# DCASE-REPO/DESED_task

Measured on AMD Instinct MI355X. Metric: 10s-clips/sec CRNN mean-teacher train @batch48, higher is better.
Workload: dtype f32 (fp32 storage and accumulation; the dense contractions of the wide layers run as split-bf16 MFMA, 3 bf16 products per fp32 product, fp32-level accuracy; everything else exact f32)

## Files before the change

### desed_task_amd/_lib.py

```python
import ctypes
import os
import re

_HERE = os.path.dirname(os.path.abspath(__file__))
_HEADER = os.path.join(os.path.dirname(_HERE), "include", "sed_hip.h")
LIB_PATH = os.path.join(_HERE, "libsed_hip.so")

_CTYPES = {"int": ctypes.c_int, "float": ctypes.c_float, "double": ctypes.c_double, "long long": ctypes.c_longlong,
           "unsigned": ctypes.c_uint, "unsigned int": ctypes.c_uint}

ERRORS = {-1: "bad argument", -2: "kernel launch failed", -3: "unsupported configuration"}


def parse_header(path=_HEADER):
    text = open(path).read()
    text = re.sub(r"/\*.*?\*/", "", text, flags=re.S)
    protos = {}
    for m in re.finditer(r"\b(?:int|long long)\s+(sed_\w+)\s*\(([^)]*)\)\s*;", text):
        args = []
        for a in m.group(2).split(","):
            a = a.strip()
            if "*" in a:
                args.append(ctypes.c_void_p)
            else:
                ty = re.sub(r"\bconst\b", "", a).strip()
                ty = ty.rsplit(None, 1)[0].strip()
                args.append(_CTYPES[ty])
        protos[m.group(1)] = args
    return protos


def header_constants(path=_HEADER):
    return {m.group(1): int(m.group(2)) for m in re.finditer(r"^#define\s+(SED_\w+)\s+(\d+)\b", open(path).read(), re.M)}


class _Lib:
    def __init__(self, path, is_emulator=False):
        self.path = path
        self.is_emulator = is_emulator
        import torch
        self._dll = ctypes.CDLL(path)
        self.protos = parse_header()
        for name, argtypes in self.protos.items():
            fn = getattr(self._dll, name)
            fn.argtypes = argtypes
            fn.restype = ctypes.c_longlong if name.endswith("_floats") else ctypes.c_int

    def value(self, name, *args):
        return getattr(self._dll, name)(*args)

    def call(self, name, *args):
        rc = getattr(self._dll, name)(*args)
        if rc != 0:
            raise RuntimeError("%s failed: %s (rc=%d)" % (name, ERRORS.get(rc, "?"), rc))


_lib = None


def get():
    global _lib
    if _lib is None:
        if not os.path.exists(LIB_PATH):
            raise RuntimeError(
                "desed_task_amd: %s is missing -- build it with `python -m desed_task_amd.build` "
                "(hipcc --offload-arch=gfx950).  There is no CPU fallback." % LIB_PATH)
        _lib = _Lib(LIB_PATH)
    return _lib


def use_library(path, is_emulator=True):
    global _lib
    _lib = _Lib(path, is_emulator=is_emulator) if path is not None else None
    return _lib


TUNING_KEYS = {"glu_grid_cap": 0, "glu_bwd128_split": 1, "convb_ck": 2, "convb_mp": 3, "block0_nocenter": 4, "glu_fwd128": 5, "wgrad_narrow": 6, "wgrad_cap": 7, "attn_valu": 8, "wgrad_wide": 9, "gru_lds_kb": 10, "mel_taps_mem": 11, "convb_tpw": 12, "mel_wave": 13, "gemm_ntn": 14, "linear_tiles": 15}


_tuning = {}


def set_tuning(key, value):
    get().call("sed_set_tuning", TUNING_KEYS[key], int(value))
    _tuning[key] = int(value)


def get_tuning(key):
    return _tuning.get(key, 0)


def check_tensor(t, name="tensor"):
    lib = get()
    if lib.is_emulator:
        if t.is_cuda:
            raise RuntimeError("%s: emulator build bound but tensor is on the GPU" % name)
    elif not t.is_cuda:
        raise RuntimeError("%s must live on the MI355X (cuda) device: there is no CPU path" % name)
    if not t.is_contiguous():
        raise RuntimeError("%s must be contiguous" % name)


def stream_ptr(t):
    if t.is_cuda:
        import torch
        return torch.cuda.current_stream(t.device).cuda_stream
    return 0
```

### desed_task_amd/csrc/sed_common.h

```cpp
#pragma once

#ifdef SED_EMU
#include "hip_emu.h"
#else
#include <hip/hip_runtime.h>
#define SED_DYN_SMEM(name) extern __shared__ __attribute__((aligned(16))) char name[]
#define SED_LAUNCH(kern, grid, block, smem, stream, ...) \
    hipLaunchKernelGGL(kern, grid, block, smem, stream, __VA_ARGS__)
typedef float f32x16 __attribute__((ext_vector_type(16)));
typedef float f32x4 __attribute__((ext_vector_type(4)));
typedef short s16x8 __attribute__((ext_vector_type(8)));
#endif

#include <stdint.h>

#define SED_API extern "C" __attribute__((visibility("default")))

#define SED_MAX_SMEM(kern, bytes) \
    (void)hipFuncSetAttribute((const void*)(kern), hipFuncAttributeMaxDynamicSharedMemorySize, (int)(bytes))

__global__ __launch_bounds__(256) static void sed_zero4_kernel(float* p0, int n0, float* p1, int n1, float* p2, int n2, float* p3, int n3) {
    const int i = blockIdx.x * 256 + threadIdx.x;
    if (i < n0) p0[i] = 0.f;
    if (i < n1) p1[i] = 0.f;
    if (i < n2) p2[i] = 0.f;
    if (i < n3) p3[i] = 0.f;
}
static inline void sed_zero4(hipStream_t s, float* p0, int n0, float* p1, int n1, float* p2, int n2, float* p3, int n3) {
    int n = n0 > n1 ? n0 : n1;
    n = n > n2 ? n : n2;
    n = n > n3 ? n : n3;
    if (n <= 0) return;
    SED_LAUNCH(sed_zero4_kernel, dim3((n + 255) / 256), dim3(256), 0, s, p0, n0, p1, n1, p2, n2, p3, n3);
}

#define SED_OK 0
#define SED_ERR_ARG (-1)
#define SED_ERR_LAUNCH (-2)
#define SED_ERR_UNSUPPORTED (-3)

enum { SED_TUNE_GLU_GRID_CAP = 0, SED_TUNE_GLU_BWD128_SPLIT = 1, SED_TUNE_CONVB_CK = 2, SED_TUNE_CONVB_MP = 3, SED_TUNE_B0_NOCENTER = 4, SED_TUNE_GLU_FWD128 = 5, SED_TUNE_WGRAD_NARROW = 6, SED_TUNE_WGRAD_CAP = 7,
       SED_TUNE_ATTN_VALU = 8, SED_TUNE_WGRAD_WIDE = 9, SED_TUNE_GRU_LDS_KB = 10, SED_TUNE_MEL_TAPS_MEM = 11, SED_TUNE_CONVB_TPW = 12, SED_TUNE_MEL_WAVE = 13, SED_TUNE_GEMM_NTN = 14, SED_TUNE_LINEAR_TILES = 15, SED_TUNE_COUNT = 16 };
extern int sed_tuning[SED_TUNE_COUNT];

static inline int sed_check_launch() {
    hipError_t e = hipGetLastError();
    return e == hipSuccess ? SED_OK : SED_ERR_LAUNCH;
}

__device__ __forceinline__ f32x16 mfma32(float a, float b, f32x16 c) {
#ifdef SED_EMU
    return emu_mfma_32x32x2(a, b, c);
#else
    return __builtin_amdgcn_mfma_f32_32x32x2f32(a, b, c, 0, 0, 0);
#endif
}
__device__ __forceinline__ int mfma32_row(int r, int lane) { return (r & 3) + 8 * (r >> 2) + 4 * (lane >> 5); }

__device__ __forceinline__ f32x4 mfma16(float a, float b, f32x4 c) {
#ifdef SED_EMU
    return emu_mfma_16x16x4(a, b, c);
#else
    return __builtin_amdgcn_mfma_f32_16x16x4f32(a, b, c, 0, 0, 0);
#endif
}

__device__ __forceinline__ f32x16 mfma32_bf16(s16x8 a, s16x8 b, f32x16 c) {
#ifdef SED_EMU
    return emu_mfma_32x32x16_bf16(a, b, c);
#else
    typedef __bf16 bf16x8_t __attribute__((ext_vector_type(8)));
    return __builtin_amdgcn_mfma_f32_32x32x16_bf16(__builtin_bit_cast(bf16x8_t, a), __builtin_bit_cast(bf16x8_t, b), c, 0, 0, 0);
#endif
}
__device__ __forceinline__ f32x4 mfma16_bf16(s16x8 a, s16x8 b, f32x4 c) {
#ifdef SED_EMU
    return emu_mfma_16x16x32_bf16(a, b, c);
#else
    typedef __bf16 bf16x8_t __attribute__((ext_vector_type(8)));
    return __builtin_amdgcn_mfma_f32_16x16x32_bf16(__builtin_bit_cast(bf16x8_t, a), __builtin_bit_cast(bf16x8_t, b), c, 0, 0, 0);
#endif
}
__device__ __forceinline__ unsigned short f32_to_bf16(float x) {
    unsigned u = __float_as_uint(x);
    u += 0x7FFFu + ((u >> 16) & 1u);
    return (unsigned short)(u >> 16);
}
__device__ __forceinline__ float bf16_to_f32(unsigned short h) { return __uint_as_float(((unsigned)h) << 16); }
__device__ __forceinline__ void bf16_split(float x, unsigned short& hi, unsigned short& lo) {
    hi = f32_to_bf16(x);
    lo = f32_to_bf16(x - bf16_to_f32(hi));
}

__device__ __forceinline__ float sed_sadd(float a, float b) {
#ifdef SED_EMU
    return a + b;
// ... 308 lines not shown
```

### desed_task_amd/csrc/sed_conv.hip

```cpp
#include "sed_common.h"

__global__ __launch_bounds__(256) void pack_weights_kernel(const float* __restrict__ W, float* __restrict__ Wf,
                                                           float* __restrict__ Wd, int COUT, int CIN) {
    const int i = blockIdx.x * 256 + threadIdx.x;
    if (i >= COUT * CIN * 9) return;
    const int b = i % 3, a = (i / 3) % 3, ci = (i / 9) % CIN, co = i / (9 * CIN);
    const float w = W[i];
    Wf[((a * 3 + b) * CIN + ci) * COUT + co] = w;
    if (Wd) Wd[(((2 - a) * 3 + (2 - b)) * COUT + co) * CIN + ci] = w;
}
SED_API int sed_conv_pack_weights(const float* W, float* Wf, float* Wd, int COUT, int CIN, void* stream) {
    const int n = COUT * CIN * 9;
    SED_LAUNCH(pack_weights_kernel, dim3((n + 255) / 256), dim3(256), 0, (hipStream_t)stream, W, Wf, Wd, COUT, CIN);
    return sed_check_launch();
}
struct PackJobs {
    const float* W[8];
    float* Wf[8];
    float* Wd[8];
    int cout[8], cin[8], start[9];
    int n;
};
__global__ __launch_bounds__(256) void pack_weights_multi_kernel(PackJobs jobs) {
    const int i = blockIdx.x * 256 + threadIdx.x;
// ... 983 lines not shown
            for (int idx = tid; idx < ntp * CIN * COUT; idx += 256) part[(size_t)g0 * CIN * COUT + idx] = red[idx];
        }
        return;
    }
#pragma unroll
    for (int g0 = 0; g0 < 9; g0 += TG) {
        for (int round = 0; round < WK; ++round) {
            __syncthreads();
            if (wk == round) {
#pragma unroll
                for (int tp = g0; tp < g0 + TG && tp < 9; ++tp)
#pragma unroll
                    for (int n = 0; n < NTW; ++n) {
                        const int co = (wn * NTW + n) * 32 + lo;
#pragma unroll
                        for (int r = 0; r < 16; ++r) {
                            const int ci = mfma32_row(r, lane);
                            if (ci < CIN) {
                                float* d = red + ((tp - g0) * CIN + ci) * COUT + co;
                                *d = (round == 0) ? acc[tp][n][r] : *d + acc[tp][n][r];
                            }
                        }
                    }
            }
        }
        __syncthreads();
        const int ntp = (9 - g0) < TG ? (9 - g0) : TG;
        for (int idx = tid; idx < ntp * CIN * COUT; idx += 256) part[(size_t)g0 * CIN * COUT + idx] = red[idx];
    }
}
template <int CIN, int COUT, int TF>
static int launch_wgrad_alltaps(const float* x, const float* dy, float* dWp, int B, int T, int F, hipStream_t s) {
    using Cfg = WgaCfg<CIN, COUT, TF>;
    const int grid = wgrad_parts(CIN, COUT, B, T, F);
    SED_MAX_SMEM((conv_wgrad_alltaps_kernel<CIN, COUT, TF>), Cfg::SMEM);
    SED_LAUNCH((conv_wgrad_alltaps_kernel<CIN, COUT, TF>), dim3(grid), dim3(256), Cfg::SMEM, s, x, dy, dWp, B, T, F);
    return sed_check_launch();
}

#ifndef WGN_ABL
#define WGN_ABL 0
#endif
template <int CIN, int COUT>
struct WgnCfg {
    static constexpr int TF = 32, TR = 4, PH = TR + 2;
    static constexpr bool M16 = CIN == 16;
    static constexpr int XS = PH * TF + (M16 ? 16 : 8), DS = TR * TF + (M16 ? 16 : 8);
    static constexpr int XPLANE = CIN * XS, DPLANE = COUT * DS;
    static constexpr int SMEM_OPS = (6 * XPLANE + 2 * DPLANE) * 2, SMEM_RED = 9 * CIN * COUT * 4;
    static constexpr int SMEM = SMEM_OPS > SMEM_RED ? SMEM_OPS : SMEM_RED;
};
template <int CIN, int COUT>
__global__ __launch_bounds__(256) void conv_wgrad_alltaps_bf16_kernel(const float* __restrict__ x, const float* __restrict__ dy,
                                                                      float* __restrict__ dWp, int B, int T, int F) {
    using Cfg = WgnCfg<CIN, COUT>;
    constexpr int TF = Cfg::TF, TR = Cfg::TR, PH = Cfg::PH, XS = Cfg::XS, DS = Cfg::DS, XPLANE = Cfg::XPLANE, DPLANE = Cfg::DPLANE;
    constexpr bool M16 = Cfg::M16;
    static_assert((CIN == 16 && COUT == 32) || (CIN == 32 && COUT == 64), "the two narrow layers of the recipe");
    SED_DYN_SMEM(smem);
    unsigned short* xp = (unsigned short*)smem;
    unsigned short* dp = xp + 6 * XPLANE;
    const int lane = threadIdx.x & 63, w = threadIdx.x >> 6;
    int tid = threadIdx.x, lo = lane & 31, hi = lane >> 5, i16 = lane & 15, g = lane >> 4;
    const int ftiles = F / TF, ttiles = (T + TR - 1) / TR, ntiles = B * ttiles * ftiles;

    f32x16 acc[M16 ? 1 : 9];
    f32x4 acc16[M16 ? 9 : 1][2];
#pragma unroll
    for (int tp = 0; tp < (M16 ? 1 : 9); ++tp) acc[tp] = f32x16_zero();
#pragma unroll
    for (int tp = 0; tp < (M16 ? 9 : 1); ++tp) { acc16[tp][0] = f32x4{0.f, 0.f, 0.f, 0.f}; acc16[tp][1] = f32x4{0.f, 0.f, 0.f, 0.f}; }

    constexpr int VX = CIN / 4, VD = COUT / 4, NXI = PH * 8 * VX, NDI = TR * 8 * VD;
    constexpr int NXU = (NXI + 255) / 256, NDU = NDI / 256;
    float4 lx[NXU][6], ld[NDU][4];
    unsigned long long okx = 0;
    unsigned okd = 0;
    static_assert(NXU * 6 <= 64 && NDU <= 32, "validity masks");
    auto load_tile = [&](int tile_) {
        const int ft = tile_ % ftiles, tt = (tile_ / ftiles) % ttiles, b = tile_ / (ftiles * ttiles);
        const int t0 = tt * TR, f0 = ft * TF;
        okx = 0; okd = 0;
#pragma unroll
        for (int u = 0; u < NXU; ++u) {
            const int it = tid + 256 * u, cq = it % 8, v = (it / 8) % VX, i = it / (8 * VX);
            const int t = t0 - 1 + i;
            const bool rowok = it < NXI && t >= 0 && t < T && !(WGN_ABL & 8);
            const float* src = x + (((size_t)b * T + (t < 0 ? 0 : (t >= T ? T - 1 : t))) * F) * CIN + 4 * v;
#pragma unroll
            for (int k = 0; k < 6; ++k) {
                const int f = f0 - 1 + 4 * cq + k;
                okx |= (unsigned long long)((rowok && f >= 0 && f < F) ? 1 : 0) << (6 * u + k);
                lx[u][k] = *(const float4*)(src + (size_t)(f < 0 ? 0 : (f >= F ? F - 1 : f)) * CIN);
            }
        }
#pragma unroll
        for (int u = 0; u < NDU; ++u) {
            const int it = tid + 256 * u, cq = it % 8, v = (it / 8) % VD, r = it / (8 * VD);
            const int t = t0 + r;
            okd |= ((t < T && !(WGN_ABL & 8)) ? 1u : 0u) << u;
            const float* src = dy + (((size_t)b * T + (t < T ? t : T - 1)) * F + f0 + 4 * cq) * COUT + 4 * v;
#pragma unroll
            for (int k = 0; k < 4; ++k) ld[u][k] = *(const float4*)(src + (size_t)k * COUT);
        }
    };
    auto comp = [](const float4& q, int c) { return c == 0 ? q.x : c == 1 ? q.y : c == 2 ? q.z : q.w; };
    auto store_tile = [&]() {
#pragma unroll
        for (int u = 0; u < NXU; ++u)
#pragma unroll
            for (int k = 0; k < 6; ++k) if (!((okx >> (6 * u + k)) & 1ull)) lx[u][k] = make_float4(0.f, 0.f, 0.f, 0.f);
#pragma unroll
        for (int u = 0; u < NDU; ++u)
            if (!((okd >> u) & 1u)) {
#pragma unroll
                for (int k = 0; k < 4; ++k) ld[u][k] = make_float4(0.f, 0.f, 0.f, 0.f);
            }
#pragma unroll
        for (int u = 0; u < NXU; ++u) {
            const int it = tid + 256 * u, cq = it % 8, v = (it / 8) % VX, i = it / (8 * VX);
            if (it < NXI) {
#pragma unroll
                for (int c = 0; c < 4; ++c) {
                    unsigned ph[5], pl[5];
#pragma unroll
                    for (int k = 0; k < 5; ++k) bf16_split2(comp(lx[u][k], c), comp(lx[u][k + 1], c), ph[k], pl[k]);
                    unsigned short* dst = xp + (4 * v + c) * XS + i * TF + 4 * cq;
#pragma unroll
                    for (int sft = 0; sft < 3; ++sft) {
                        uint2 hv, lv;
                        hv.x = ph[sft]; hv.y = ph[sft + 2];
                        lv.x = pl[sft]; lv.y = pl[sft + 2];
                        *(uint2*)(dst + (2 * sft) * XPLANE) = hv;
                        *(uint2*)(dst + (2 * sft + 1) * XPLANE) = lv;
                    }
                }
            }
        }
#pragma unroll
        for (int u = 0; u < NDU; ++u) {
            const int it = tid + 256 * u, cq = it % 8, v = (it / 8) % VD, r = it / (8 * VD);
#pragma unroll
            for (int c = 0; c < 4; ++c) {
                uint2 hv, lv;
                bf16_split2(comp(ld[u][0], c), comp(ld[u][1], c), hv.x, lv.x);
                bf16_split2(comp(ld[u][2], c), comp(ld[u][3], c), hv.y, lv.y);
                unsigned short* dst = dp + (4 * v + c) * DS + r * TF + 4 * cq;
                *(uint2*)dst = hv;
                *(uint2*)(dst + DPLANE) = lv;
            }
        }
    };
    int tile = blockIdx.x;
    if (tile < ntiles) load_tile(tile);
    for (; tile < ntiles; tile += gridDim.x) {
        sed_opaque(tid); sed_opaque(lo); sed_opaque(hi); sed_opaque(i16); sed_opaque(g);
        __syncthreads();
        if (!(WGN_ABL & 4)) store_tile();
        else if (lx[0][0].x + ld[0][0].x == 123.456f) xp[tid] = 1;
        __syncthreads();
        if (tile + (int)gridDim.x < ntiles) load_tile(tile + gridDim.x);
        if (WGN_ABL & 2) continue;
        if (M16) {
            s16x8 bh[2], bl[2], ah[9], al[9];
#pragma unroll
            for (int nt = 0; nt < 2; ++nt) {
                const unsigned short* bp = dp + (16 * nt + i16) * DS + w * TF + 8 * g;
                bh[nt] = *(const s16x8*)bp;
                bl[nt] = *(const s16x8*)(bp + DPLANE);
            }
#pragma unroll
            for (int tp = 0; tp < 9; ++tp) {
                const unsigned short* ap = xp + (2 * (tp % 3)) * XPLANE + i16 * XS + (w + tp / 3) * TF + 8 * g;
                ah[tp] = *(const s16x8*)ap;
                al[tp] = *(const s16x8*)(ap + XPLANE);
            }
            sed_sched_fence();
#pragma unroll
            for (int tp = 0; tp < 9; ++tp)
#pragma unroll
                for (int nt = 0; nt < 2; ++nt) {
                    f32x4 a = acc16[M16 ? tp : 0][nt];
                    if (WGN_ABL & 1) { a[0] += (float)(al[tp][0] + bh[nt][1] + ah[tp][2] + bl[nt][3]); }
                    else {
                    a = mfma16_bf16(al[tp], bh[nt], a);
                    a = mfma16_bf16(ah[tp], bl[nt], a);
                    a = mfma16_bf16(ah[tp], bh[nt], a);
                    }
                    acc16[M16 ? tp : 0][nt] = a;
                }
        } else {
            const int wn = w & 1, wk = w >> 1;
            s16x8 bh[2], bl[2], ah[2][9], al[2][9];
            auto fetch = [&](int k4, int buf) {
                const int ks = 4 * wk + k4, r = ks >> 1, c0 = 16 * (ks & 1) + 8 * hi;
                const unsigned short* bp = dp + (32 * wn + lo) * DS + r * TF + c0;
                bh[buf] = *(const s16x8*)bp;
                bl[buf] = *(const s16x8*)(bp + DPLANE);
#pragma unroll
                for (int tp = 0; tp < 9; ++tp) {
                    const unsigned short* ap = xp + (2 * (tp % 3)) * XPLANE + lo * XS + (r + tp / 3) * TF + c0;
                    ah[buf][tp] = *(const s16x8*)ap;
                    al[buf][tp] = *(const s16x8*)(ap + XPLANE);
                }
            };
            fetch(0, 0);
            sed_sched_fence();
#pragma unroll
            for (int k4 = 0; k4 < 4; ++k4) {
                const int cur = k4 & 1;
                if (k4 + 1 < 4) fetch(k4 + 1, cur ^ 1);
#pragma unroll
                for (int tp = 0; tp < 9; ++tp) {
                    f32x16 a = acc[M16 ? 0 : tp];
                    if (WGN_ABL & 1) { a[0] += (float)(al[cur][tp][0] + bh[cur][1] + ah[cur][tp][2] + bl[cur][3]); }
                    else {
                    a = mfma32_bf16(al[cur][tp], bh[cur], a);
                    a = mfma32_bf16(ah[cur][tp], bl[cur], a);
                    a = mfma32_bf16(ah[cur][tp], bh[cur], a);
                    }
                    acc[M16 ? 0 : tp] = a;
                }
                sed_sched_fence();
            }
        }
    }
    float* red = (float*)smem;
    float* part = dWp + (size_t)blockIdx.x * 9 * CIN * COUT;
    if (M16) {
        for (int round = 0; round < 4; ++round) {
            __syncthreads();
            if (w == round) {
#pragma unroll
                for (int tp = 0; tp < 9; ++tp)
#pragma unroll
                    for (int nt = 0; nt < 2; ++nt)
#pragma unroll
                        for (int r = 0; r < 4; ++r) {
                            float* d = red + (tp * CIN + 4 * g + r) * COUT + 16 * nt + i16;
                            const float v = acc16[M16 ? tp : 0][nt][r];
                            *d = round == 0 ? v : *d + v;
                        }
            }
        }
    } else {
        const int wn = w & 1, wk = w >> 1;
        for (int round = 0; round < 2; ++round) {
            __syncthreads();
            if (wk == round) {
#pragma unroll
                for (int tp = 0; tp < 9; ++tp)
#pragma unroll
                    for (int r = 0; r < 16; ++r) {
                        float* d = red + (tp * CIN + mfma32_row(r, lane)) * COUT + 32 * wn + lo;
                        const float v = acc[M16 ? 0 : tp][r];
                        *d = round == 0 ? v : *d + v;
                    }
            }
        }
    }
    __syncthreads();
    for (int idx = threadIdx.x; idx < 9 * CIN * COUT; idx += 256) part[idx] = red[idx];
}
template <int CIN, int COUT>
static int launch_wgrad_alltaps_bf16(const float* x, const float* dy, float* dWp, int B, int T, int F, int grid, hipStream_t s) {
    using Cfg = WgnCfg<CIN, COUT>;
    SED_MAX_SMEM((conv_wgrad_alltaps_bf16_kernel<CIN, COUT>), Cfg::SMEM);
    SED_LAUNCH((conv_wgrad_alltaps_bf16_kernel<CIN, COUT>), dim3(grid), dim3(256), Cfg::SMEM, s, x, dy, dWp, B, T, F);
    return sed_check_launch();
}

static int conv_wgrad_impl(const float* x, const float* dy, float* dWp, float* dW, int B, int T, int F, int CIN, int COUT,
                           bool split_bf16, void* stream) {
    hipStream_t s = (hipStream_t)stream;
    int rc = SED_ERR_UNSUPPORTED;
    const int TF = conv_tf(F);
    if (F % TF != 0 || (F & (F - 1)) != 0) return SED_ERR_UNSUPPORTED;
    int nparts = wgrad_parts(CIN, COUT, B, T, F);
    if (split_bf16 && TF == 32 && sed_tuning[SED_TUNE_WGRAD_NARROW] != 1 && ((CIN == 16 && COUT == 32) || (CIN == 32 && COUT == 64))) {
        const int capb = sed_tuning[SED_TUNE_WGRAD_CAP] > 0 ? sed_tuning[SED_TUNE_WGRAD_CAP] : (CIN == 16 ? 512 : 256);
        if (nparts > capb) nparts = capb;
        if (CIN == 16) rc = launch_wgrad_alltaps_bf16<16, 32>(x, dy, dWp, B, T, F, nparts, s);
        else rc = launch_wgrad_alltaps_bf16<32, 64>(x, dy, dWp, B, T, F, nparts, s);
    }
#define WGA_CASE(ci, co, tf) if (rc != SED_OK && CIN == ci && COUT == co && TF == tf) rc = launch_wgrad_alltaps<ci, co, tf>(x, dy, dWp, B, T, F, s);
    WGA_CASE(16, 32, 32) WGA_CASE(16, 32, 16) WGA_CASE(16, 32, 8) WGA_CASE(32, 64, 32) WGA_CASE(32, 64, 16) WGA_CASE(32, 64, 8)
    WGA_CASE(32, 64, 4)
#undef WGA_CASE
    if (rc != SED_OK && split_bf16 && wgrad_row_ok(CIN, COUT, F) && sed_tuning[SED_TUNE_WGRAD_WIDE] != 1) {
        nparts = wgrad_row_parts(CIN, B, T, F);
        if (CIN == 64) rc = launch_wgrad_bf16_row<64, 128, 128>(x, dy, dWp, B, T, F, nparts, s);
        else rc = launch_wgrad_bf16_row<128, 128, 64>(x, dy, dWp, B, T, F, nparts, s);
    }
#define WG_CASE(ci, co)                                                                                        \
    if (rc != SED_OK && CIN == ci && COUT == co)                                                               \
        rc = split_bf16 ? launch_wgrad_bf16<ci, co>(x, dy, dWp, B, T, F, s) : launch_wgrad<ci, co>(x, dy, dWp, B, T, F, s);
    WG_CASE(64, 128) WG_CASE(128, 128)
#undef WG_CASE
    if (rc != SED_OK) return rc;
    const int n = COUT * CIN * 9;
    SED_LAUNCH(wgrad_reduce_kernel, dim3((n + 63) / 64), dim3(nparts >= 256 ? 1024 : 256), 0, s, (const float*)dWp, dW, nparts, COUT, CIN);
    return sed_check_launch();
}
SED_API int sed_conv_wgrad(const float* x, const float* dy, float* dWp, float* dW, int B, int T, int F, int CIN, int COUT,
                              void* stream) {
    return conv_wgrad_impl(x, dy, dWp, dW, B, T, F, CIN, COUT, false, stream);
}
SED_API int sed_conv_wgrad_bf16x3(const float* x, const float* dy, float* dWp, float* dW, int B, int T, int F, int CIN,
                                     int COUT, void* stream) {
    return conv_wgrad_impl(x, dy, dWp, dW, B, T, F, CIN, COUT, true, stream);
}

__global__ __launch_bounds__(256) void conv0_wgrad_kernel(const float* __restrict__ x, const int* __restrict__ bounds,
                                                          const float* __restrict__ dyz, const float* __restrict__ y,
                                                          const float* __restrict__ stats, const float* __restrict__ gamma,
                                                          const float* __restrict__ dgamma, const float* __restrict__ dbeta,
                                                          float* __restrict__ dW, int B, int T, int F, int tiles_t, int fuse_bn,
                                                          int training, float inv_count) {
    constexpr int C = 16;
    __shared__ float tile[(C0_TR + 2) * (128 + 2)];
    __shared__ float red[4][144];
// ... 83 lines not shown
```

### desed_task_amd/csrc/sed_conv_bf16.hip

```cpp
#include "sed_common.h"
#include <stdlib.h>

#define CONVB_THREADS(COUT) ((COUT) >= 64 ? 512 : 256)

template <int CIN, int COUT, int TF, int MP = 128, int CKT = 32>
struct ConvBCfg {
    static constexpr int TR = MP / TF;
#ifdef CONVB_OLDMAP
    static constexpr int PWL = TF + 2, PW = TF + 2, PH = TR + 2, PP = PW * PH, PPL = PWL * PH;
#else
    static constexpr int PWL = TF + 2, PW = TF == 8 ? 12 : (TF == 2 ? 6 : TF + 2), PH = TR + 2, PP = PW * PH, PPL = PWL * PH;
#endif
    static constexpr int CK = CIN < CKT ? CIN : CKT;
    static constexpr int RSS = CK + 8;
    static constexpr int NCH = CIN / CK;
    static constexpr int NT = (COUT + 31) / 32;
    static constexpr int NCOL = NT * 32;
    static constexpr int WM = MP / 32;
    static constexpr int THREADS = CONVB_THREADS(COUT);
    static constexpr int WN = THREADS / 64 / WM;
    static constexpr int NTW = NT / WN;
    static_assert(NTW >= 1 && NTW * WN == NT, "wave split must tile COUT");
    static_assert(THREADS % (CK / 4) == 0, "a thread keeps one channel quad for all its patch elements");
    static constexpr int PATCH_S = 2 * PP * RSS;
// ... 97 lines not shown
                                     int* bounds, int B, int nb, int f_param, int n_freq, int t_param, int n_time, unsigned seed,
                                     const unsigned* seed_dev, const float* copy_src, float* copy_dst, long long copy_n, void* stream) {
    if (n < 0 || n > 8) return SED_ERR_ARG;
    if (bounds && B > 0 && nb != 1 && nb != B) return SED_ERR_ARG;
    if (copy_dst && (!copy_src || copy_n < 0 || ((uintptr_t)copy_src & 15) || ((uintptr_t)copy_dst & 15))) return SED_ERR_ARG;
    PackBJobs jobs;
    const int tot = packb_jobs(jobs, n, W, Wf, Wd, cout, cin) * (packb_any_dgrad(jobs) ? 2 : 1);
    PrologueExtra ex;
    ex.bounds = (bounds && B > 0) ? bounds : nullptr; ex.B = B; ex.nb = nb; ex.f_param = f_param; ex.n_freq = n_freq;
    ex.t_param = t_param; ex.n_time = n_time; ex.seed = (uint32_t)seed; ex.seed_dev = seed_dev;
    const size_t n4 = copy_dst ? (size_t)copy_n / 4 : 0;
    ex.src = (const float4*)copy_src; ex.dst = (float4*)copy_dst; ex.n4 = n4;
    ex.ntail = copy_dst ? (int)(copy_n % 4) : 0;
    ex.src_tail = copy_src ? copy_src + 4 * n4 : nullptr; ex.dst_tail = copy_dst ? copy_dst + 4 * n4 : nullptr;
    ex.pack_blocks = (tot + 255) / 256;
    size_t cb = (n4 + 1023) / 1024;
    ex.copy_blocks = (int)(cb > 4096 ? 4096 : cb);
    if (ex.pack_blocks == 0 && !ex.bounds && n4 == 0 && ex.ntail == 0) return SED_OK;
    SED_LAUNCH(cnn_prologue_bf16_kernel, dim3(ex.pack_blocks + 1 + ex.copy_blocks), dim3(256), 0, (hipStream_t)stream, jobs, ex);
    return sed_check_launch();
}

#ifndef CONVB_ABL
#define CONVB_ABL 0
#endif

struct ConvBnb {
    const float* ybn;
    const float* stats;
    const float* gamma;
    const float* dgamma;
    const float* dbeta;
    float* dy_out;
    float* dbias;
    float inv_count;
};

template <int TF>
__device__ __forceinline__ void conv_lane_pixel(int i, int& prow, int& pcol) {
    if (TF >= 32) { prow = 0; pcol = i; return; }
#ifdef CONVB_OLDMAP
    prow = i / TF; pcol = i % TF; return;
#endif
    const int qd = i >> 2, gsel = (0x96 >> qd) & 1, g = 4 * (qd >> 1) + (i & 3);
    if (TF == 2) { prow = 8 * gsel + (g >> 1); pcol = g & 1; }
    else { prow = gsel + 2 * (g / TF); pcol = g % TF; }
}

template <int CIN, int COUT, int TF, bool STATS, int MP = 128, int CKT = 32, bool BNB = false>
__global__ __launch_bounds__(CONVB_THREADS(COUT)) void conv3x3_bf16_kernel(const float* __restrict__ x,
                                                                            const unsigned short* __restrict__ Wp,
                                                                            const float* __restrict__ bias, float* __restrict__ y,
                                                                            float* __restrict__ partial, int B, int T, int F,
                                                                            ConvBnb bnb) {
    using Cfg = ConvBCfg<CIN, COUT, TF, MP, CKT>;
    constexpr int TR = Cfg::TR, PW = Cfg::PW, PWL = Cfg::PWL, PP = Cfg::PP, PPL = Cfg::PPL, CK = Cfg::CK, RSS = Cfg::RSS, NCH = Cfg::NCH, NT = Cfg::NT,
                  NTW = Cfg::NTW, THREADS = Cfg::THREADS, WM = Cfg::WM, NCOL = Cfg::NCOL, SLAB = Cfg::SLAB, WBUF_S = Cfg::WBUF_S;
    SED_DYN_SMEM(smem_raw);
    unsigned short* patch = (unsigned short*)smem_raw;
    unsigned short* wbuf = patch + Cfg::PATCH_S;
    float* bnc = (float*)(smem_raw + Cfg::SMEM);
    const int tid = threadIdx.x, lane = tid & 63, w = (tid >> 6) % WM, wn = (tid >> 6) / WM, lo = lane & 31, hi = lane >> 5;
    const int ftiles = F / TF, ttiles = (T + TR - 1) / TR, ntiles = B * ttiles * ftiles;
    constexpr int WROWS = TF >= 32 ? 1 : 32 / TF;
    int lprow, lpcol;
    conv_lane_pixel<TF>(lo, lprow, lpcol);
    const int abase = (((TF >= 32 ? (32 * w) / TF : WROWS * w) + lprow) * PW + (TF >= 32 ? (32 * w) % TF : 0) + lpcol) * RSS + 8 * hi;

    f32x16 acc[NTW];

    if (NCOL > COUT) {
        for (int i = tid; i < 3 * WBUF_S; i += THREADS) wbuf[i] = 0;
        __syncthreads();
    }
    constexpr int WPIECES = SLAB / 8;
    constexpr int WV = (WPIECES + THREADS - 1) / THREADS;
    constexpr int V = CK / 4;
    constexpr int NLD = (PPL * V + THREADS - 1) / THREADS;
    uint4 wreg[3 * WV];
    float4 ld[NLD];
    float4 ldy[BNB ? NLD : 1];
    if (BNB) {
        for (int c = tid; c < CIN; c += THREADS) {
            const float g = bnb.gamma[c];
            bnc[c] = bnb.stats[c];
            bnc[CIN + c] = bnb.stats[CIN + c];
            bnc[2 * CIN + c] = g * bnb.dbeta[c] * bnb.inv_count;
            bnc[3 * CIN + c] = g * bnb.dgamma[c] * bnb.inv_count;
        }
        if (blockIdx.x == 0 && tid < CIN && bnb.dbias != nullptr) bnb.dbias[tid] = 0.f;
        __syncthreads();
    }
    auto w_dst = [&](int buf, int piece) -> unsigned short* {
        const int plane = piece / (COUT * CK / 8), rem = piece - plane * (COUT * CK / 8);
        const int co = rem / (CK / 8), pc = rem - co * (CK / 8);
        return wbuf + buf * WBUF_S + plane * NCOL * RSS + co * RSS + 8 * pc;
    };
    auto load_row = [&](int cc, int r) {
#pragma unroll
        for (int t3 = 0; t3 < 3; ++t3) {
            const uint4* src = (const uint4*)(Wp + ((size_t)(3 * r + t3) * NCH + cc) * SLAB);
#pragma unroll
            for (int i = 0; i < WV; ++i) {
                const int piece = tid + THREADS * i;
                uint4 v = make_uint4(0u, 0u, 0u, 0u);
                if (piece < WPIECES && !(CONVB_ABL & 1)) v = src[piece];
                wreg[t3 * WV + i] = v;
            }
        }
    };
    auto store_row = [&]() {
#pragma unroll
        for (int t3 = 0; t3 < 3; ++t3)
#pragma unroll
            for (int i = 0; i < WV; ++i) {
                const int piece = tid + THREADS * i;
                if (piece < WPIECES) *(uint4*)w_dst(t3, piece) = wreg[t3 * WV + i];
            }
    };
    auto load_patch = [&](int cc, int pb, int pt0, int pf0) {
#pragma unroll
        for (int u = 0; u < NLD; ++u) {
            const int idx = tid + THREADS * u;
            const int pix = idx / V, v = idx - pix * V;
            const int i = pix / PWL, j = pix - i * PWL;
            const int t = pt0 - 1 + i, f = pf0 - 1 + j;
            ld[u] = make_float4(0.f, 0.f, 0.f, 0.f);
            if (BNB) ldy[u] = make_float4(0.f, 0.f, 0.f, 0.f);
            if (idx < PPL * V && t >= 0 && t < T && f >= 0 && f < F && !(CONVB_ABL & 4)) {
                const size_t off = (((size_t)pb * T + t) * F + f) * CIN + cc * CK + 4 * v;
                ld[u] = *(const float4*)(x + off);
                if (BNB) ldy[u] = *(const float4*)(bnb.ybn + off);
            }
        }
    };
    constexpr bool PERS = CIN <= 32;
    bool primed = false;
    int tile_it = blockIdx.x;
    do {
    const int tile = PERS ? tile_it : (int)blockIdx.x;
    const int ft = tile % ftiles, tt = (tile / ftiles) % ttiles, b = tile / (ftiles * ttiles);
    const int t0 = tt * TR, f0 = ft * TF;
    const int tile_n = PERS ? tile + (int)gridDim.x : ntiles;
    int nb = 0, nt0 = 0, nf0 = 0;
    if (PERS && tile_n < ntiles) { nb = tile_n / (ftiles * ttiles); nt0 = ((tile_n / ftiles) % ttiles) * TR; nf0 = (tile_n % ftiles) * TF; }
    auto store_patch = [&](int cc) {
        float4 bmean, bistd, bm1, bm2;
        if (BNB) {
            const int c0 = cc * CK + 4 * (tid % V);
            bmean = *(const float4*)(bnc + c0);
            bistd = *(const float4*)(bnc + CIN + c0);
            bm1 = *(const float4*)(bnc + 2 * CIN + c0);
            bm2 = *(const float4*)(bnc + 3 * CIN + c0);
        }
#pragma unroll
        for (int u = 0; u < NLD; ++u) {
            const int idx = tid + THREADS * u;
            if (idx < PPL * V) {
                const int pixl = idx / V, v = idx - pixl * V;
                const int i = pixl / PWL, j = pixl - i * PWL, pix = i * PW + j;
                if (BNB) {
                    const int t = t0 - 1 + i, f = f0 - 1 + j;
                    if (t >= 0 && t < T && f >= 0 && f < F) {
                        float4 g = ld[u];
                        const float4 yv = ldy[u];
                        g.x = bistd.x * (g.x - bm1.x - (yv.x - bmean.x) * bistd.x * bm2.x);
                        g.y = bistd.y * (g.y - bm1.y - (yv.y - bmean.y) * bistd.y * bm2.y);
                        g.z = bistd.z * (g.z - bm1.z - (yv.z - bmean.z) * bistd.z * bm2.z);
                        g.w = bistd.w * (g.w - bm1.w - (yv.w - bmean.w) * bistd.w * bm2.w);
                        ld[u] = g;
                        if (i >= 1 && i <= TR && j >= 1 && j <= TF)
                            *(float4*)(bnb.dy_out + (((size_t)b * T + t) * F + f) * CIN + cc * CK + 4 * v) = g;
                    }
                }
                uint2 hv, lv;
                bf16_split2(ld[u].x, ld[u].y, hv.x, lv.x);
                bf16_split2(ld[u].z, ld[u].w, hv.y, lv.y);
                *(uint2*)(patch + pix * RSS + 4 * v) = hv;
                *(uint2*)(patch + PP * RSS + pix * RSS + 4 * v) = lv;
            }
        }
    };

#pragma unroll
    for (int nt = 0; nt < NTW; ++nt) acc[nt] = f32x16_zero();
    if (!PERS || !primed) {
        load_patch(0, b, t0, f0);
        load_row(0, 0);
        primed = true;
    }
    store_patch(0);
    store_row();
    __syncthreads();
#pragma unroll 1
    for (int cc = 0; cc < NCH; ++cc) {
#pragma unroll
        for (int r = 0; r < 3; ++r) {
            const bool next_chunk = r == 2 && cc + 1 < NCH;
            const bool more = r < 2 || cc + 1 < NCH;
            if (more) load_row(r < 2 ? cc : cc + 1, r < 2 ? r + 1 : 0);
            if (next_chunk) load_patch(cc + 1, b, t0, f0);
            if (PERS && !more && tile_n < ntiles) {
                load_row(0, 0);
                load_patch(0, nb, nt0, nf0);
            }
#pragma unroll
            for (int t3 = 0; t3 < 3; ++t3) {
                const unsigned short* wb = wbuf + t3 * WBUF_S;
                const unsigned short* ap = patch + abase + (r * PW + t3) * RSS;
#pragma unroll
                for (int ks = 0; ks < CK / 16; ++ks) {
                    s16x8 a_hi, a_lo;
                    if (CONVB_ABL & 16) { a_hi = (s16x8)(short)(lane + ks); a_lo = (s16x8)(short)(lane + t3); }
                    else { a_hi = *(const s16x8*)(ap + 16 * ks); a_lo = *(const s16x8*)(ap + PP * RSS + 16 * ks); }
#pragma unroll
                    for (int nt = 0; nt < NTW; ++nt) {
                        const unsigned short* bp = wb + ((wn * NTW + nt) * 32 + lo) * RSS + 16 * ks + 8 * hi;
                        s16x8 b_hi, b_lo;
                        if (CONVB_ABL & 16) { b_hi = (s16x8)(short)(lane + nt); b_lo = (s16x8)(short)(lane + r); }
                        else { b_hi = *(const s16x8*)bp; b_lo = *(const s16x8*)(bp + NCOL * RSS); }
                        if (CONVB_ABL & 2) { acc[nt][0] += (float)(a_lo[0] + b_hi[0] + a_hi[1] + b_lo[1]); continue; }
                        acc[nt] = mfma32_bf16(a_lo, b_hi, acc[nt]);
                        acc[nt] = mfma32_bf16(a_hi, b_lo, acc[nt]);
                        acc[nt] = mfma32_bf16(a_hi, b_hi, acc[nt]);
                    }
                }
            }
            if (!(CONVB_ABL & 8)) __syncthreads();
            if (more) store_row();
            if (next_chunk) store_patch(cc + 1);
            if (!(CONVB_ABL & 8)) __syncthreads();
        }
    }
    float* red = (float*)wbuf;
#pragma unroll
    for (int nt = 0; nt < NTW; ++nt) {
        const int co = (wn * NTW + nt) * 32 + lo;
        const float bv = (bias != nullptr && co < COUT) ? bias[co] : 0.f;
        float s = 0.f, s2 = 0.f;
#pragma unroll
        for (int r = 0; r < 16; ++r) {
            int eprow, epcol;
            conv_lane_pixel<TF>(mfma32_row(r, lane), eprow, epcol);
            const int t = t0 + (TF >= 32 ? (32 * w) / TF : WROWS * w) + eprow, f = f0 + (TF >= 32 ? (32 * w) % TF : 0) + epcol;
            if (t < T && co < COUT) {
                const float v = acc[nt][r] + bv;
                if (!(CONVB_ABL & 32)) y[(((size_t)b * T + t) * F + f) * COUT + co] = v;
                s += v;
                s2 += v * v;
            }
        }
        if (STATS) {
            s += __shfl_xor(s, 32);
            s2 += __shfl_xor(s2, 32);
            if (hi == 0) {
                red[(w * 2 + 0) * (NT * 32) + co] = s;
                red[(w * 2 + 1) * (NT * 32) + co] = s2;
            }
        }
    }
    if (STATS) {
        __syncthreads();
        if (tid < 2 * COUT) {
            const int which = tid / COUT, co = tid - which * COUT;
            float v = 0.f;
#pragma unroll
            for (int ww = 0; ww < WM; ++ww) v += red[(ww * 2 + which) * (NT * 32) + co];
            partial[(size_t)tid * ntiles + tile] = v;
        }
    }
    if (PERS && STATS && NCOL > COUT) {
        __syncthreads();
        for (int i = tid; i < 3 * WBUF_S; i += THREADS) wbuf[i] = 0;
    }
    if constexpr (!PERS) break;
    __syncthreads();
    tile_it += (int)gridDim.x;
    } while (tile_it < ntiles);
}

template <class K>
static inline int convb_persistent_grid(K kern, int threads, int smem, int ntiles, int CIN) {
    if (CIN > 32) return ntiles;
    const int e = sed_tuning[SED_TUNE_CONVB_TPW];
    if (e < 0) return ntiles;
    if (e > 0) return (ntiles + e - 1) / e;
#ifdef SED_EMU
    (void)kern; (void)threads; (void)smem;
    return ntiles;
#else
    static int slots = 0;
    if (slots == 0) {
        int per_cu = 0, dev = 0;
        hipDeviceProp_t prop;
        if (hipGetDevice(&dev) != hipSuccess || hipGetDeviceProperties(&prop, dev) != hipSuccess ||
            hipOccupancyMaxActiveBlocksPerMultiprocessor(&per_cu, (const void*)kern, threads, (size_t)smem) != hipSuccess || per_cu < 1)
            slots = -1;
        else
            slots = per_cu * prop.multiProcessorCount;
    }
    if (slots < 0 || ntiles <= 2 * slots) return ntiles;
    return slots;
#endif
}

template <int CIN, int COUT, int TF, int MP = 128, int CKT = 32, bool BNB = false>
static int launch_convb(const float* x, const unsigned short* Wp, const float* bias, float* y, float* partial, int B, int T, int F,
                        hipStream_t s, ConvBnb bnb = ConvBnb()) {
    using Cfg = ConvBCfg<CIN, COUT, TF, MP, CKT>;
    const int ntiles = B * ((T + Cfg::TR - 1) / Cfg::TR) * (F / TF);
    if constexpr (BNB) {
        if constexpr (CIN >= COUT) {
            SED_MAX_SMEM((conv3x3_bf16_kernel<CIN, COUT, TF, false, MP, CKT, true>), Cfg::SMEM_BNB);
            const int nblk = convb_persistent_grid(conv3x3_bf16_kernel<CIN, COUT, TF, false, MP, CKT, true>, Cfg::THREADS, Cfg::SMEM_BNB, ntiles, CIN);
            SED_LAUNCH((conv3x3_bf16_kernel<CIN, COUT, TF, false, MP, CKT, true>), dim3(nblk), dim3(Cfg::THREADS), Cfg::SMEM_BNB, s, x, Wp, bias, y, partial, B, T, F, bnb);
            return sed_check_launch();
        } else {
            return SED_ERR_UNSUPPORTED;
        }
    } else if (partial) {
        SED_MAX_SMEM((conv3x3_bf16_kernel<CIN, COUT, TF, true, MP, CKT>), Cfg::SMEM);
        const int nblk = convb_persistent_grid(conv3x3_bf16_kernel<CIN, COUT, TF, true, MP, CKT>, Cfg::THREADS, Cfg::SMEM, ntiles, CIN);
        SED_LAUNCH((conv3x3_bf16_kernel<CIN, COUT, TF, true, MP, CKT>), dim3(nblk), dim3(Cfg::THREADS), Cfg::SMEM, s, x, Wp, bias, y, partial, B, T, F, bnb);
    } else {
        SED_MAX_SMEM((conv3x3_bf16_kernel<CIN, COUT, TF, false, MP, CKT>), Cfg::SMEM);
        const int nblk = convb_persistent_grid(conv3x3_bf16_kernel<CIN, COUT, TF, false, MP, CKT>, Cfg::THREADS, Cfg::SMEM, ntiles, CIN);
        SED_LAUNCH((conv3x3_bf16_kernel<CIN, COUT, TF, false, MP, CKT>), dim3(nblk), dim3(Cfg::THREADS), Cfg::SMEM, s, x, Wp, bias, y, partial, B, T, F, bnb);
    }
    return sed_check_launch();
}

static inline int convb_mp(int F, int CIN, int COUT) {
    const int e = sed_tuning[SED_TUNE_CONVB_MP];
    if (e && COUT >= 64) return e;
    if (COUT < 64) return 128;
    if (CIN <= 32) return 128;
    if (CIN == 128 && COUT == 128 && F <= 2) return 64;
    if (CIN == 128 && COUT == 128 && F <= 4) return 128;
    return 256;
}
SED_API int sed_conv_fwd_blocks_bf16(int B, int T, int F, int CIN, int COUT) {
    if (CIN == 1) return B * ((T + 15) / 16);
    const int TF = F >= 32 ? 32 : F;
    const int TR = convb_mp(F, CIN, COUT) / TF;
    return B * ((T + TR - 1) / TR) * (F / TF);
}

template <bool BNB>
static int convb_dispatch(const float* x, const void* Wp, const float* bias, float* y, float* partial, int B, int T, int F,
                          int CIN, int COUT, hipStream_t s, ConvBnb bnb) {
    if (B <= 0 || T <= 0) return SED_OK;
    const int TF = F >= 32 ? 32 : F;
    if (F % TF != 0 || (F & (F - 1)) != 0 || F < 2) return SED_ERR_UNSUPPORTED;
    const unsigned short* W = (const unsigned short*)Wp;
    const int MP = convb_mp(F, CIN, COUT);
    const int CK = CIN >= 32 ? convb_ck(CIN, COUT) : 32;
#define CONVB_CASE16(ci, co, tf, mp) \
    if (CIN == ci && COUT == co && TF == tf && MP == mp && CK == 16) return launch_convb<ci, co, tf, mp, 16, BNB>(x, W, bias, y, partial, B, T, F, s, bnb);
    CONVB_CASE16(32, 64, 32, 128) CONVB_CASE16(64, 128, 16, 128) CONVB_CASE16(64, 128, 16, 256)
    CONVB_CASE16(128, 128, 8, 128) CONVB_CASE16(128, 128, 8, 256) CONVB_CASE16(128, 128, 4, 64) CONVB_CASE16(128, 128, 4, 128)
    CONVB_CASE16(128, 128, 2, 64) CONVB_CASE16(128, 128, 2, 128) CONVB_CASE16(64, 32, 32, 128)
    CONVB_CASE16(128, 64, 16, 128) CONVB_CASE16(128, 64, 16, 256)
    CONVB_CASE16(64, 128, 4, 256) CONVB_CASE16(64, 128, 8, 256) CONVB_CASE16(64, 128, 32, 256)
    CONVB_CASE16(128, 64, 4, 256) CONVB_CASE16(128, 64, 8, 256) CONVB_CASE16(128, 64, 32, 256)
#undef CONVB_CASE16
    if (CK == 16) return SED_ERR_UNSUPPORTED;
#define CONVB_CASE(ci, co, tf, mp) \
    if (CIN == ci && COUT == co && TF == tf && MP == mp) return launch_convb<ci, co, tf, mp, 32, BNB>(x, W, bias, y, partial, B, T, F, s, bnb);
    CONVB_CASE(16, 32, 32, 128)
    CONVB_CASE(32, 64, 32, 128) CONVB_CASE(32, 64, 32, 256)
    CONVB_CASE(64, 128, 16, 128) CONVB_CASE(64, 128, 16, 256)
    CONVB_CASE(128, 128, 8, 128) CONVB_CASE(128, 128, 8, 256)
    CONVB_CASE(128, 128, 4, 64) CONVB_CASE(128, 128, 4, 128) CONVB_CASE(128, 128, 4, 256)
    CONVB_CASE(128, 128, 2, 64) CONVB_CASE(128, 128, 2, 128)
    CONVB_CASE(32, 16, 32, 128) CONVB_CASE(64, 32, 32, 128)
    CONVB_CASE(128, 64, 16, 128) CONVB_CASE(128, 64, 16, 256)
    CONVB_CASE(16, 32, 16, 128) CONVB_CASE(32, 64, 8, 256) CONVB_CASE(32, 64, 16, 256) CONVB_CASE(64, 128, 4, 256) CONVB_CASE(64, 128, 8, 256)
    CONVB_CASE(64, 128, 32, 256) CONVB_CASE(128, 128, 16, 256) CONVB_CASE(128, 128, 32, 256)
    CONVB_CASE(32, 16, 16, 128) CONVB_CASE(64, 32, 8, 128) CONVB_CASE(64, 32, 16, 128) CONVB_CASE(128, 64, 4, 256) CONVB_CASE(128, 64, 8, 256)
    CONVB_CASE(128, 64, 32, 256)
// ... 19 lines not shown
```

Before: 16390.

## Walk conv tiles in contiguous per-XCD strips and slide the halo rows between tiles

Persistent conv3x3 bf16 blocks now take a contiguous strip of tiles along time, ordered with an XCD-aware rank, instead of striding across the grid. When the next tile directly follows in time, the kernel copies the two overlapping halo rows inside LDS and loads only the new rows, which cuts global loads. The wgrad all-taps kernel also remaps block slots by XCD rank to improve L2 locality. The new walk is on by default and can be turned off with a tuning key. It adds index bookkeeping and an LDS copy per tile, and strips of uneven length may leave the load less balanced.

```diff
diff --git a/desed_task_amd/_lib.py b/desed_task_amd/_lib.py
--- a/desed_task_amd/_lib.py
+++ b/desed_task_amd/_lib.py
@@ -75,7 +75,7 @@
     return _lib
 
 
-TUNING_KEYS = {"glu_grid_cap": 0, "glu_bwd128_split": 1, "convb_ck": 2, "convb_mp": 3, "block0_nocenter": 4, "glu_fwd128": 5, "wgrad_narrow": 6, "wgrad_cap": 7, "attn_valu": 8, "wgrad_wide": 9, "gru_lds_kb": 10, "mel_taps_mem": 11, "convb_tpw": 12, "mel_wave": 13, "gemm_ntn": 14, "linear_tiles": 15}
+TUNING_KEYS = {"glu_grid_cap": 0, "glu_bwd128_split": 1, "convb_ck": 2, "convb_mp": 3, "block0_nocenter": 4, "glu_fwd128": 5, "wgrad_narrow": 6, "wgrad_cap": 7, "attn_valu": 8, "wgrad_wide": 9, "gru_lds_kb": 10, "mel_taps_mem": 11, "convb_tpw": 12, "mel_wave": 13, "gemm_ntn": 14, "linear_tiles": 15, "conv_walk": 16}
 
 
 _tuning = {}
diff --git a/desed_task_amd/csrc/sed_common.h b/desed_task_amd/csrc/sed_common.h
--- a/desed_task_amd/csrc/sed_common.h
+++ b/desed_task_amd/csrc/sed_common.h
@@ -40,8 +40,13 @@
 #define SED_ERR_UNSUPPORTED (-3)
 
 enum { SED_TUNE_GLU_GRID_CAP = 0, SED_TUNE_GLU_BWD128_SPLIT = 1, SED_TUNE_CONVB_CK = 2, SED_TUNE_CONVB_MP = 3, SED_TUNE_B0_NOCENTER = 4, SED_TUNE_GLU_FWD128 = 5, SED_TUNE_WGRAD_NARROW = 6, SED_TUNE_WGRAD_CAP = 7,
-       SED_TUNE_ATTN_VALU = 8, SED_TUNE_WGRAD_WIDE = 9, SED_TUNE_GRU_LDS_KB = 10, SED_TUNE_MEL_TAPS_MEM = 11, SED_TUNE_CONVB_TPW = 12, SED_TUNE_MEL_WAVE = 13, SED_TUNE_GEMM_NTN = 14, SED_TUNE_LINEAR_TILES = 15, SED_TUNE_COUNT = 16 };
+       SED_TUNE_ATTN_VALU = 8, SED_TUNE_WGRAD_WIDE = 9, SED_TUNE_GRU_LDS_KB = 10, SED_TUNE_MEL_TAPS_MEM = 11, SED_TUNE_CONVB_TPW = 12, SED_TUNE_MEL_WAVE = 13, SED_TUNE_GEMM_NTN = 14, SED_TUNE_LINEAR_TILES = 15, SED_TUNE_CONV_WALK = 16, SED_TUNE_COUNT = 17 };
 extern int sed_tuning[SED_TUNE_COUNT];
+
+__host__ __device__ __forceinline__ int sed_xcd_rank(int g, int G) {
+    const int x = g & 7, q = G >> 3, r = G & 7;
+    return x * q + (x < r ? x : r) + (g >> 3);
+}
 
 static inline int sed_check_launch() {
     hipError_t e = hipGetLastError();
diff --git a/desed_task_amd/csrc/sed_conv.hip b/desed_task_amd/csrc/sed_conv.hip
--- a/desed_task_amd/csrc/sed_conv.hip
+++ b/desed_task_amd/csrc/sed_conv.hip
@@ -1059,7 +1059,7 @@
 };
 template <int CIN, int COUT>
 __global__ __launch_bounds__(256) void conv_wgrad_alltaps_bf16_kernel(const float* __restrict__ x, const float* __restrict__ dy,
-                                                                      float* __restrict__ dWp, int B, int T, int F) {
+                                                                      float* __restrict__ dWp, int B, int T, int F, int walk) {
     using Cfg = WgnCfg<CIN, COUT>;
     constexpr int TF = Cfg::TF, TR = Cfg::TR, PH = Cfg::PH, XS = Cfg::XS, DS = Cfg::DS, XPLANE = Cfg::XPLANE, DPLANE = Cfg::DPLANE;
     constexpr bool M16 = Cfg::M16;
@@ -1158,7 +1158,8 @@
             }
         }
     };
-    int tile = blockIdx.x;
+    const int slot = walk == 0 ? sed_xcd_rank(blockIdx.x, gridDim.x) : (int)blockIdx.x;
+    int tile = slot;
     if (tile < ntiles) load_tile(tile);
     for (; tile < ntiles; tile += gridDim.x) {
         sed_opaque(tid); sed_opaque(lo); sed_opaque(hi); sed_opaque(i16); sed_opaque(g);
@@ -1233,7 +1234,7 @@
         }
     }
     float* red = (float*)smem;
-    float* part = dWp + (size_t)blockIdx.x * 9 * CIN * COUT;
+    float* part = dWp + (size_t)slot * 9 * CIN * COUT;
     if (M16) {
         for (int round = 0; round < 4; ++round) {
             __syncthreads();
@@ -1273,7 +1274,8 @@
 static int launch_wgrad_alltaps_bf16(const float* x, const float* dy, float* dWp, int B, int T, int F, int grid, hipStream_t s) {
     using Cfg = WgnCfg<CIN, COUT>;
     SED_MAX_SMEM((conv_wgrad_alltaps_bf16_kernel<CIN, COUT>), Cfg::SMEM);
-    SED_LAUNCH((conv_wgrad_alltaps_bf16_kernel<CIN, COUT>), dim3(grid), dim3(256), Cfg::SMEM, s, x, dy, dWp, B, T, F);
+    SED_LAUNCH((conv_wgrad_alltaps_bf16_kernel<CIN, COUT>), dim3(grid), dim3(256), Cfg::SMEM, s, x, dy, dWp, B, T, F,
+               sed_tuning[SED_TUNE_CONV_WALK] == 1 ? 1 : 0);
     return sed_check_launch();
 }
 
diff --git a/desed_task_amd/csrc/sed_conv_bf16.hip b/desed_task_amd/csrc/sed_conv_bf16.hip
--- a/desed_task_amd/csrc/sed_conv_bf16.hip
+++ b/desed_task_amd/csrc/sed_conv_bf16.hip
@@ -173,9 +173,9 @@
                                                                             const unsigned short* __restrict__ Wp,
                                                                             const float* __restrict__ bias, float* __restrict__ y,
                                                                             float* __restrict__ partial, int B, int T, int F,
-                                                                            ConvBnb bnb) {
+                                                                            ConvBnb bnb, int walk) {
     using Cfg = ConvBCfg<CIN, COUT, TF, MP, CKT>;
-    constexpr int TR = Cfg::TR, PW = Cfg::PW, PWL = Cfg::PWL, PP = Cfg::PP, PPL = Cfg::PPL, CK = Cfg::CK, RSS = Cfg::RSS, NCH = Cfg::NCH, NT = Cfg::NT,
+    constexpr int TR = Cfg::TR, PH = Cfg::PH, PW = Cfg::PW, PWL = Cfg::PWL, PP = Cfg::PP, PPL = Cfg::PPL, CK = Cfg::CK, RSS = Cfg::RSS, NCH = Cfg::NCH, NT = Cfg::NT,
                   NTW = Cfg::NTW, THREADS = Cfg::THREADS, WM = Cfg::WM, NCOL = Cfg::NCOL, SLAB = Cfg::SLAB, WBUF_S = Cfg::WBUF_S;
     SED_DYN_SMEM(smem_raw);
     unsigned short* patch = (unsigned short*)smem_raw;
@@ -231,41 +231,61 @@
         }
     };
     auto store_row = [&]() {
+        int tq = tid;
+        if (CIN <= 32) sed_opaque(tq);
 #pragma unroll
         for (int t3 = 0; t3 < 3; ++t3)
 #pragma unroll
             for (int i = 0; i < WV; ++i) {
-                const int piece = tid + THREADS * i;
+                const int piece = tq + THREADS * i;
                 if (piece < WPIECES) *(uint4*)w_dst(t3, piece) = wreg[t3 * WV + i];
             }
     };
-    auto load_patch = [&](int cc, int pb, int pt0, int pf0) {
+    constexpr bool PERS = CIN <= 32;
+    auto load_patch = [&](int cc, int pb, int pt0, int pf0, int row0) {
+        int tq = tid;
+        if (PERS) sed_opaque(tq);
 #pragma unroll
         for (int u = 0; u < NLD; ++u) {
-            const int idx = tid + THREADS * u;
+            const int idx = tq + THREADS * u;
             const int pix = idx / V, v = idx - pix * V;
-            const int i = pix / PWL, j = pix - i * PWL;
+            const int i = pix / PWL + row0, j = pix % PWL;
             const int t = pt0 - 1 + i, f = pf0 - 1 + j;
             ld[u] = make_float4(0.f, 0.f, 0.f, 0.f);
             if (BNB) ldy[u] = make_float4(0.f, 0.f, 0.f, 0.f);
-            if (idx < PPL * V && t >= 0 && t < T && f >= 0 && f < F && !(CONVB_ABL & 4)) {
+            if (i < PH && t >= 0 && t < T && f >= 0 && f < F && !(CONVB_ABL & 4)) {
                 const size_t off = (((size_t)pb * T + t) * F + f) * CIN + cc * CK + 4 * v;
                 ld[u] = *(const float4*)(x + off);
                 if (BNB) ldy[u] = *(const float4*)(bnb.ybn + off);
             }
         }
     };
-    constexpr bool PERS = CIN <= 32;
-    bool primed = false;
-    int tile_it = blockIdx.x;
+    constexpr bool SLIDE = PERS && NCH == 1 && TR >= 2;
+    const bool strips = walk == 0;
+    const int grid = (int)gridDim.x;
+    int wi = blockIdx.x, wend = ntiles, wstep = grid;
+    if (strips) {
+        const int v = sed_xcd_rank(blockIdx.x, grid), q = ntiles / grid, r = ntiles - q * grid;
+        wi = v * q + (v < r ? v : r);
+        wend = wi + q + (v < r ? 1 : 0);
+        wstep = 1;
+    }
+    if (wi >= wend) return;
+    auto locate = [&](int wi_, int& b_, int& tt_, int& ft_) {
+        if (strips) { const int sp = wi_ / ttiles; tt_ = wi_ - sp * ttiles; b_ = sp / ftiles; ft_ = sp - b_ * ftiles; }
+        else { ft_ = wi_ % ftiles; tt_ = (wi_ / ftiles) % ttiles; b_ = wi_ / (ftiles * ttiles); }
+    };
+    bool primed = false, slide = false;
     do {
-    const int tile = PERS ? tile_it : (int)blockIdx.x;
-    const int ft = tile % ftiles, tt = (tile / ftiles) % ttiles, b = tile / (ftiles * ttiles);
+    int b, tt, ft;
+    locate(wi, b, tt, ft);
+    const int tile = (b * ttiles + tt) * ftiles + ft;
     const int t0 = tt * TR, f0 = ft * TF;
-    const int tile_n = PERS ? tile + (int)gridDim.x : ntiles;
+    const bool has_next = PERS && wi + wstep < wend;
     int nb = 0, nt0 = 0, nf0 = 0;
-    if (PERS && tile_n < ntiles) { nb = tile_n / (ftiles * ttiles); nt0 = ((tile_n / ftiles) % ttiles) * TR; nf0 = (tile_n % ftiles) * TF; }
-    auto store_patch = [&](int cc) {
+    if (has_next) { int ntt, nft; locate(wi + wstep, nb, ntt, nft); nt0 = ntt * TR; nf0 = nft * TF; }
+    const bool slide_n = SLIDE && strips && has_next && nb == b && nf0 == f0 && nt0 == t0 + TR;
+    auto store_patch = [&](int cc, int row0) {
         float4 bmean, bistd, bm1, bm2;
         if (BNB) {
             const int c0 = cc * CK + 4 * (tid % V);
@@ -274,12 +294,14 @@
             bm1 = *(const float4*)(bnc + 2 * CIN + c0);
             bm2 = *(const float4*)(bnc + 3 * CIN + c0);
         }
+        int tq = tid;
+        if (PERS) sed_opaque(tq);
 #pragma unroll
         for (int u = 0; u < NLD; ++u) {
-            const int idx = tid + THREADS * u;
-            if (idx < PPL * V) {
-                const int pixl = idx / V, v = idx - pixl * V;
-                const int i = pixl / PWL, j = pixl - i * PWL, pix = i * PW + j;
+            const int idx = tq + THREADS * u;
+            const int pixl = idx / V, v = idx - pixl * V;
+            const int i = pixl / PWL + row0, j = pixl % PWL, pix = i * PW + j;
+            if (i < PH) {
                 if (BNB) {
                     const int t = t0 - 1 + i, f = f0 - 1 + j;
                     if (t >= 0 && t < T && f >= 0 && f < F) {
@@ -290,7 +312,7 @@
                         g.z = bistd.z * (g.z - bm1.z - (yv.z - bmean.z) * bistd.z * bm2.z);
                         g.w = bistd.w * (g.w - bm1.w - (yv.w - bmean.w) * bistd.w * bm2.w);
                         ld[u] = g;
-                        if (i >= 1 && i <= TR && j >= 1 && j <= TF)
+                        if (i >= 1 && i <= TR + (slide_n ? 1 : 0) && j >= 1 && j <= TF)
                             *(float4*)(bnb.dy_out + (((size_t)b * T + t) * F + f) * CIN + cc * CK + 4 * v) = g;
                     }
                 }
@@ -306,11 +328,11 @@
 #pragma unroll
     for (int nt = 0; nt < NTW; ++nt) acc[nt] = f32x16_zero();
     if (!PERS || !primed) {
-        load_patch(0, b, t0, f0);
+        load_patch(0, b, t0, f0, 0);
         load_row(0, 0);
         primed = true;
     }
-    store_patch(0);
+    store_patch(0, SLIDE && slide ? 2 : 0);
     store_row();
     __syncthreads();
 #pragma unroll 1
@@ -320,10 +342,10 @@
             const bool next_chunk = r == 2 && cc + 1 < NCH;
             const bool more = r < 2 || cc + 1 < NCH;
             if (more) load_row(r < 2 ? cc : cc + 1, r < 2 ? r + 1 : 0);
-            if (next_chunk) load_patch(cc + 1, b, t0, f0);
-            if (PERS && !more && tile_n < ntiles) {
+            if (next_chunk) load_patch(cc + 1, b, t0, f0, 0);
+            if (PERS && !more && has_next) {
                 load_row(0, 0);
-                load_patch(0, nb, nt0, nf0);
+                load_patch(0, nb, nt0, nf0, slide_n ? 2 : 0);
             }
 #pragma unroll
             for (int t3 = 0; t3 < 3; ++t3) {
@@ -349,7 +371,7 @@
             }
             if (!(CONVB_ABL & 8)) __syncthreads();
             if (more) store_row();
-            if (next_chunk) store_patch(cc + 1);
+            if (next_chunk) store_patch(cc + 1, 0);
             if (!(CONVB_ABL & 8)) __syncthreads();
         }
     }
@@ -395,9 +417,18 @@
         for (int i = tid; i < 3 * WBUF_S; i += THREADS) wbuf[i] = 0;
     }
     if constexpr (!PERS) break;
+    if (SLIDE && slide_n) {
+        constexpr int RP = 2 * PW * RSS / 8;
+#pragma unroll 1
+        for (int i = tid; i < 2 * RP; i += THREADS) {
+            unsigned short* d = patch + (i >= RP ? PP * RSS : 0) + 8 * (i >= RP ? i - RP : i);
+            *(uint4*)d = *(const uint4*)(d + TR * PW * RSS);
+        }
+    }
     __syncthreads();
-    tile_it += (int)gridDim.x;
-    } while (tile_it < ntiles);
+    slide = slide_n;
+    wi += wstep;
+    } while (wi < wend);
 }
 
 template <class K>
@@ -430,11 +461,12 @@
                         hipStream_t s, ConvBnb bnb = ConvBnb()) {
     using Cfg = ConvBCfg<CIN, COUT, TF, MP, CKT>;
     const int ntiles = B * ((T + Cfg::TR - 1) / Cfg::TR) * (F / TF);
+    const int walk = sed_tuning[SED_TUNE_CONV_WALK] == 1 ? 1 : 0;
     if constexpr (BNB) {
         if constexpr (CIN >= COUT) {
             SED_MAX_SMEM((conv3x3_bf16_kernel<CIN, COUT, TF, false, MP, CKT, true>), Cfg::SMEM_BNB);
             const int nblk = convb_persistent_grid(conv3x3_bf16_kernel<CIN, COUT, TF, false, MP, CKT, true>, Cfg::THREADS, Cfg::SMEM_BNB, ntiles, CIN);
-            SED_LAUNCH((conv3x3_bf16_kernel<CIN, COUT, TF, false, MP, CKT, true>), dim3(nblk), dim3(Cfg::THREADS), Cfg::SMEM_BNB, s, x, Wp, bias, y, partial, B, T, F, bnb);
+            SED_LAUNCH((conv3x3_bf16_kernel<CIN, COUT, TF, false, MP, CKT, true>), dim3(nblk), dim3(Cfg::THREADS), Cfg::SMEM_BNB, s, x, Wp, bias, y, partial, B, T, F, bnb, walk);
             return sed_check_launch();
         } else {
             return SED_ERR_UNSUPPORTED;
@@ -442,11 +474,11 @@
     } else if (partial) {
         SED_MAX_SMEM((conv3x3_bf16_kernel<CIN, COUT, TF, true, MP, CKT>), Cfg::SMEM);
         const int nblk = convb_persistent_grid(conv3x3_bf16_kernel<CIN, COUT, TF, true, MP, CKT>, Cfg::THREADS, Cfg::SMEM, ntiles, CIN);
-        SED_LAUNCH((conv3x3_bf16_kernel<CIN, COUT, TF, true, MP, CKT>), dim3(nblk), dim3(Cfg::THREADS), Cfg::SMEM, s, x, Wp, bias, y, partial, B, T, F, bnb);
+        SED_LAUNCH((conv3x3_bf16_kernel<CIN, COUT, TF, true, MP, CKT>), dim3(nblk), dim3(Cfg::THREADS), Cfg::SMEM, s, x, Wp, bias, y, partial, B, T, F, bnb, walk);
     } else {
         SED_MAX_SMEM((conv3x3_bf16_kernel<CIN, COUT, TF, false, MP, CKT>), Cfg::SMEM);
         const int nblk = convb_persistent_grid(conv3x3_bf16_kernel<CIN, COUT, TF, false, MP, CKT>, Cfg::THREADS, Cfg::SMEM, ntiles, CIN);
-        SED_LAUNCH((conv3x3_bf16_kernel<CIN, COUT, TF, false, MP, CKT>), dim3(nblk), dim3(Cfg::THREADS), Cfg::SMEM, s, x, Wp, bias, y, partial, B, T, F, bnb);
+        SED_LAUNCH((conv3x3_bf16_kernel<CIN, COUT, TF, false, MP, CKT>), dim3(nblk), dim3(Cfg::THREADS), Cfg::SMEM, s, x, Wp, bias, y, partial, B, T, F, bnb, walk);
     }
     return sed_check_launch();
 }
```

Result: no change. 16310 (-0.5%).
